# danini/progressive-x

Measured on AMD Instinct MI355X. Metric: residual_evals_per_sec, higher is better.
Workload: dtype f64; 1 GPU; C4 multi-6D-pose points (1e6 2D-3D correspondences, 16 objects, 20% outliers) x metric batch of 2048 pose hypotheses (16 GT + perturbed; weak mode: per GPU), PnP reprojection residual, MSAC + compound-model score, compound instance = 1 model; points=1000000, points_per_gpu=1000000, hypotheses_per_gpu=2048, hypotheses_total=2048, parallelism=1 GPU, exchange=none, device=AMD GPU, 256 CUs (gfx950:sramecc+:xnack-), cu_count=256

## Files before the change

### progressive-x_amd/csrc/score.hip

```cpp
#include <cmath>
#include <cstdlib>

#include "pgx_internal.h"
#include "score_filters.hip.h"
#include "score_runs.h"

namespace pgx {


template <int MT, bool MASK, int FILT>
__global__ __launch_bounds__(kScoreBlock) void score_kernel(
    const double* __restrict__ pts, int64_t n, const double* __restrict__ models, int M, int Mpad,
    double T2, const double* __restrict__ comp, int has_comp, int64_t chunk,
    const double* __restrict__ pmax, double guard, const float* __restrict__ pts32, double guard32,
    unsigned* __restrict__ pcnt, double* __restrict__ pval, double* __restrict__ psh,
    unsigned long long* __restrict__ masks, int64_t words, const int* __restrict__ perm, int chunks, int xcd_map,
    const float* __restrict__ gbounds)
{
    using R = Residual<MT>;
    int gx = (int)blockIdx.x, gy = (int)blockIdx.y;
    if (xcd_map) {
        const int groups = Mpad / kScoreBlock;
        const int slot = (int)(blockIdx.x >> 3);
        gx = slot % groups;
// ... 19 lines not shown
    const float Tup32 = f32_up(sqrt(T2) * (1.0 + 1.0 / 64.0));

    unsigned cnt = 0;
    double val = 0.0, sh = 0.0;
    unsigned long long word = 0;

    auto step = [&](int64_t i, const double (&pt)[R::D], double pm, const float* p32) {
        bool inl = false;
        bool rejected = false;
        if (FILT == 1 && F::enabled) rejected = F::reject(pt, mdl, flane, pm, T2d);
        if (FILT == 2 && F32::enabled) rejected = F32::reject(p32, flane32, T2d32);
        if (live && !rejected) {
            const double sq = R::squared(pt, mdl);
            inl = sq < T2;
            if (inl) {
                ++cnt;
                const double s = cv_max(0.0, 1.0 - sq / T2);
                val += s;
                if (has_comp) sh += cv_min(comp[i], s);
            }
        }
        if (MASK) {
            word |= (unsigned long long)(inl ? 1 : 0) << (i & 63);
            if ((i & 63) == 63 || i == i1 - 1) {
                if (live) masks[(int64_t)perm[m] * words + (i >> 6)] = word;
                word = 0;
            }
        }
    };
    constexpr int kUnroll = 4;
    int64_t i = i0;
    while (i < i1) {
        const int64_t gend = ((i | 63) + 1 < i1) ? (i | 63) + 1 : i1;
        if (FILT == 2 && F32::enabled && gbounds != nullptr) {
            const float* __restrict__ g = gbounds + (i >> 6) * kGroupRow;
            float gr[kGroupRow];
#pragma unroll
            for (int k = 0; k < 9; ++k) gr[k] = g[k];
            const bool keep = live && !F32::group_reject(gr, flane32, Tup32);
            if (__ballot(keep) == 0) {
                if (MASK && live) masks[(int64_t)perm[m] * words + (i >> 6)] = 0;
                i = gend;
                continue;
            }
        }
        for (; i + kUnroll <= gend; i += kUnroll) {
            const double* __restrict__ prow = pts + i * R::D;
            double pt[kUnroll][R::D];
            double pm[kUnroll];
            float p32[kUnroll][8];
#pragma unroll
            for (int u = 0; u < kUnroll; ++u) {
#pragma unroll
                for (int k = 0; k < R::D; ++k) pt[u][k] = prow[u * R::D + k];
                pm[u] = (FILT == 1 && F::enabled) ? pmax[i + u] : 1.0;
                if (FILT == 2 && F32::enabled) {
#pragma unroll
                    for (int k = 0; k < 8; ++k) p32[u][k] = pts32[(i + u) * 8 + k];
                }
            }
#pragma unroll
            for (int u = 0; u < kUnroll; ++u) step(i + u, pt[u], pm[u], p32[u]);
        }
        for (; i < gend; ++i) {
            const double* __restrict__ prow = pts + i * R::D;
            double pt[R::D];
            float p32[8];
#pragma unroll
            for (int k = 0; k < R::D; ++k) pt[k] = prow[k];
            if (FILT == 2 && F32::enabled) {
#pragma unroll
                for (int k = 0; k < 8; ++k) p32[k] = pts32[i * 8 + k];
            }
            step(i, pt, (FILT == 1 && F::enabled) ? pmax[i] : 1.0, p32);
        }
    }
    const int64_t o = (int64_t)gy * Mpad + m;
    pcnt[o] = cnt;
    pval[o] = val;
    psh[o] = sh;
}

#ifndef PGX_SCORE_TRIM
#define PGX_SCORE_TRIM 7
#endif
constexpr bool kTrimRows = (PGX_SCORE_TRIM & 1) != 0, kTrimDrain = (PGX_SCORE_TRIM & 2) != 0, kTrimDirect = (PGX_SCORE_TRIM & 4) != 0;

template <int MT> struct HypRow {
    using LaneT = typename Filter32<MT>::Lane;
    static_assert(sizeof(LaneT) % sizeof(float) == 0, "Filter32 lane constants are floats");
    static constexpr int kLaneVals = (int)(sizeof(LaneT) / sizeof(float));
    static constexpr int kVals = kTrimRows ? StagedVals<Filter32<MT>>::value : kLaneVals;
    static_assert(kVals <= kLaneVals, "the staged form is a prefix of the lane");
    static constexpr int kChunks = (kVals + 3) / 4;
    static constexpr int kStride = 4 * kChunks;

    static __device__ __forceinline__ void store(const LaneT& ln, float* __restrict__ row)
    {
        const float* src = reinterpret_cast<const float*>(&ln);
#pragma unroll
        for (int k = 0; k < kVals; ++k) row[k] = src[k];
    }
    static __device__ __forceinline__ LaneT load(const float* __restrict__ row)
    {
        LaneT ln;
        float* dst = reinterpret_cast<float*>(&ln);
#pragma unroll
        for (int k = 0; k < kVals; ++k) dst[k] = row[k];
        return ln;
    }
    static __device__ __forceinline__ void stage(const float* __restrict__ row0, float (*lds)[64][4], int lane)
    {
        const float* __restrict__ row = static_cast<const float*>(__builtin_assume_aligned(row0, 16));
#pragma unroll
        for (int c = 0; c < kChunks; ++c) {
            if (4 * c + 4 <= kVals) {
                *reinterpret_cast<float4*>(&lds[c][lane][0]) = *reinterpret_cast<const float4*>(row + 4 * c);
            } else {
#pragma unroll
                for (int k = 0; k < kVals - 4 * c; ++k) lds[c][lane][k] = row[4 * c + k];
            }
        }
    }
    static __device__ __forceinline__ LaneT staged(const float (*lds)[64][4], int h)
    {
        LaneT ln;
        float* dst = reinterpret_cast<float*>(&ln);
#pragma unroll
        for (int c = 0; c < kChunks; ++c) {
            if (4 * c + 4 <= kVals) {
                const float4 v = *reinterpret_cast<const float4*>(&lds[c][h][0]);
                dst[4 * c] = v.x; dst[4 * c + 1] = v.y; dst[4 * c + 2] = v.z; dst[4 * c + 3] = v.w;
            } else {
#pragma unroll
                for (int k = 0; k < kVals - 4 * c; ++k) dst[4 * c + k] = lds[c][h][k];
            }
        }
        return ln;
    }
};

constexpr int kCullWaves = 4;
constexpr int kCullTile = 64;

template <int MT>
__global__ __launch_bounds__(64 * kCullWaves) void score_cull_kernel(
    const double* __restrict__ models, int M, double T2, double guard32, const float* __restrict__ gbounds, int groups,
    int gps , int W, unsigned long long* __restrict__ keep, float* __restrict__ hyp32,
    double* __restrict__ models_t ,
    unsigned long long* __restrict__ zero , int64_t zero_words)
{
    using R = Residual<MT>;
    using F32 = Filter32<MT>;
    __shared__ __attribute__((aligned(16))) float s_gb[kCullTile + kCullTile / kSuper][kGroupRow];
    {
        const int64_t nthreads = (int64_t)gridDim.x * gridDim.y * (64 * kCullWaves);
        for (int64_t i = ((int64_t)blockIdx.y * gridDim.x + blockIdx.x) * (64 * kCullWaves) + threadIdx.x; i < zero_words; i += nthreads) zero[i] = 0ull;
    }
    const int lane = (int)(threadIdx.x & 63);
    const int w = (int)blockIdx.x * kCullWaves + (int)(threadIdx.x >> 6), seg = (int)blockIdx.y;
    const int m = w * 64 + lane;
    const bool live = w < W && m < M;
    double mdl[R::P];
#pragma unroll
    for (int k = 0; k < R::P; ++k) mdl[k] = live ? models[(int64_t)m * R::P + k] : __builtin_nan("");
    const typename F32::Lane flane32 = F32::prep(mdl, guard32, T2);
    if (seg == 0 && w < W) {
        HypRow<MT>::store(flane32, hyp32 + (int64_t)m * HypRow<MT>::kStride);
#pragma unroll
        for (int k = 0; k < R::P; ++k) models_t[(int64_t)k * W * 64 + m] = mdl[k];
    }
    const float Tup32 = f32_up(sqrt(T2) * (1.0 + 1.0 / 64.0));
    const int g0 = seg * gps, g1 = g0 + gps < groups ? g0 + gps : groups;
    for (int t0 = g0; t0 < g1; t0 += kCullTile) {
        const int cnt = g1 - t0 < kCullTile ? g1 - t0 : kCullTile;
        __syncthreads();
        const int scnt = (cnt + kSuper - 1) / kSuper;
        for (int e = (int)threadIdx.x; e < cnt * kGroupRow; e += 64 * kCullWaves)
            (&s_gb[0][0])[e] = gbounds[(int64_t)t0 * kGroupRow + e];
        for (int e = (int)threadIdx.x; e < scnt * kGroupRow; e += 64 * kCullWaves)
            (&s_gb[kCullTile][0])[e] = gbounds[((int64_t)groups + t0 / kSuper) * kGroupRow + e];
        __syncthreads();
        if (w >= W) continue;
        for (int sgi = 0; sgi < scnt; ++sgi) {
            const int i0 = sgi * kSuper, i1 = i0 + kSuper < cnt ? i0 + kSuper : cnt;
            float sr[kGroupRow];
#pragma unroll
            for (int k = 0; k < F32::kGroupVals; ++k) sr[k] = s_gb[kCullTile + sgi][k];
            if (__ballot(live && !F32::group_reject(sr, flane32, Tup32)) == 0) {
                if (lane < i1 - i0) keep[(int64_t)(t0 + i0 + lane) * W + w] = 0;
                continue;
            }
            for (int i = i0; i < i1; ++i) {
                float gr[kGroupRow];
#pragma unroll
                for (int k = 0; k < F32::kGroupVals; ++k) gr[k] = s_gb[i][k];
                const unsigned long long bm = __ballot(live && !F32::group_reject(gr, flane32, Tup32));
                if (lane == 0) keep[(int64_t)(t0 + i) * W + w] = bm;
            }
        }
    }
}

__device__ __forceinline__ long long to_fixed(double x)
{
    const double magic = 6755399441055744.0;
    return __double_as_longlong(x + magic) - __double_as_longlong(magic);
}

constexpr int kGroupWaves = 1;

template <int MT, bool MASK, bool STATS = false>
__global__ __launch_bounds__(64 * kGroupWaves) void score_group_kernel(
    const double* __restrict__ pts, const float* __restrict__ pts32, const double* __restrict__ comp, int64_t n, int groups,
    const double* __restrict__ models, int W, double T2, int has_comp, const unsigned long long* __restrict__ keep,
    const float* __restrict__ hyp32, double qscale, unsigned long long* __restrict__ acc ,
    int Mpad, unsigned long long* __restrict__ masks, int64_t words, const int* __restrict__ perm, int split, int xcd_local, const double* __restrict__ models_t,
    unsigned long long* __restrict__ stats ,
    const double* __restrict__ pts_g ,
    const float* __restrict__ p32_g , int nrep, int dense_min)
{
    using R = Residual<MT>;
    using F32 = Filter32<MT>;
    using LaneT = typename F32::Lane;
    using Row = HypRow<MT>;
    const int lane = (int)(threadIdx.x & 63);
    const int wv = 0;
    int g, part;
    if (xcd_local) {
        const int slot = (int)(blockIdx.x >> 3);
        g = (slot / split) * 8 + (int)(blockIdx.x & 7u);
        part = slot % split;
        if (g >= groups) return;
    } else {
        g = (int)blockIdx.x / split;
        part = (int)blockIdx.x % split;
    }
    g = __builtin_amdgcn_readfirstlane(g);
    part = __builtin_amdgcn_readfirstlane(part);
    {
        unsigned long long any = 0;
        for (int w = part; w < W; w += split) any |= keep[(int64_t)g * W + w];
        if (any == 0) return;
    }
    const int64_t j = (int64_t)g * 64 + lane;
    const bool valid = j < n;
    const int64_t jj = valid ? j : n - 1;
    double pt[R::D];
    float p32[8];
    if (pts_g != nullptr) {
#pragma unroll
        for (int q = 0; q < R::D; ++q) pt[q] = pts_g[((int64_t)g * R::D + q) * 64 + lane];
#pragma unroll
        for (int q = 0; q < 8; ++q) p32[q] = 0.0f;
        if constexpr (R::in1 >= R::in0) {
#pragma unroll
            for (int q = 0; q < R::D; ++q) p32[q] = (float)pt[q];
            double pm = 1.0;
#pragma unroll
            for (int q = R::in0; q <= R::in1; ++q) { const double a = fabs(pt[q]); if (!(a <= pm)) pm = a; }
            p32[5] = (float)(pm * 1.000001);
        } else {
#pragma unroll
            for (int q = 0; q < F32::kRowVals; ++q) p32[q] = p32_g[((int64_t)g * 8 + q) * 64 + lane];
        }
    } else {
#pragma unroll
        for (int q = 0; q < R::D; ++q) pt[q] = pts[jj * R::D + q];
#pragma unroll
        for (int q = 0; q < 8; ++q) p32[q] = pts32[jj * 8 + q];
    }
    const double cmp = has_comp ? comp[jj] : 0.0;
    acc += (size_t)(blockIdx.x % (unsigned)nrep) * 3 * (size_t)Mpad;
    const float T2d32 = f32_up(T2 * (1.0 + kFilter32Delta));
    __shared__ __attribute__((aligned(16))) float s_h32[kGroupWaves][Row::kChunks][64][4];
    __shared__ unsigned s_queue[kGroupWaves][128];
    int qn = 0;
    unsigned long long st_steps = 0, st_exact = 0, st_inl = 0;
    auto drain = [&](int c) __attribute__((always_inline)) {
        const bool act = lane < c;
        const unsigned e = act ? s_queue[wv][lane] : 0u;
        const int m = act ? (int)(e >> 6) : -1 - lane;
        const int src = act ? (int)(e & 63u) : lane;
        double q_pt[R::D];
#pragma unroll
        for (int k = 0; k < R::D; ++k) q_pt[k] = __shfl(pt[k], src, 64);
        const double q_cmp = has_comp ? __shfl(cmp, src, 64) : 0.0;
        long long cnt = 0, val = 0, shq = 0;
        if (act) {
            double mdl[R::P];
#pragma unroll
            for (int k = 0; k < R::P; ++k) mdl[k] = models_t[(int64_t)k * Mpad + m];
            const double sq = R::squared(q_pt, mdl);
            if (STATS) ++st_exact;
            if (sq < T2) {
                const double sc = cv_max(0.0, 1.0 - sq / T2);
                cnt = 1;
                if (STATS) ++st_inl;
                val = to_fixed(sc * qscale);
                if (has_comp) shq = to_fixed(cv_min(q_cmp, sc) * qscale);
            }
        }
        const int mp = __shfl_up(m, 1, 64);
        const bool head = lane == 0 || mp != m;
        if constexpr (kTrimDrain) {
            const int dist = run_dist(__ballot(head), lane);
            unsigned long long pv = run_pack((unsigned)cnt, (unsigned long long)val);
#pragma unroll 1
            for (int off = 1; off < 64; off <<= 1) {
                const bool same = off < dist;
                if (__ballot(same) == 0) break;
                const unsigned long long p2 = __shfl_down(pv, off, 64);
                if (same) pv += p2;
                if (has_comp) {
                    const long long s2 = __shfl_down(shq, off, 64);
                    if (same) shq += s2;
                }
            }
            cnt = (long long)run_count(pv);
            val = (long long)run_value(pv);
        } else {
            for (int off = 1; off < 64; off <<= 1) {
                const int mo = __shfl_down(m, off, 64);
                const bool same = lane + off < 64 && mo == m;
                if (__ballot(same) == 0) break;
                const long long c2 = __shfl_down(cnt, off, 64), v2 = __shfl_down(val, off, 64), s2 = __shfl_down(shq, off, 64);
                if (same) { cnt += c2; val += v2; shq += s2; }
            }
        }
        if (act && head && cnt > 0) {
            atomicAdd(&acc[m], (unsigned long long)cnt);
            atomicAdd(&acc[(int64_t)Mpad + m], (unsigned long long)val);
            if (has_comp) atomicAdd(&acc[2 * (int64_t)Mpad + m], (unsigned long long)shq);
        }
    };
    auto direct = [&](int m, bool cand) __attribute__((always_inline)) {
        double sc = 0.0, shv = 0.0;
        bool inl = false;
        if (cand) {
            double mdl[R::P];
#pragma unroll
            for (int k = 0; k < R::P; ++k) mdl[k] = models[(int64_t)m * R::P + k];
            const double sq = R::squared(pt, mdl);
            inl = sq < T2;
            if (STATS) { ++st_exact; if (inl) ++st_inl; }
            if (inl) {
                sc = cv_max(0.0, 1.0 - sq / T2);
                if (has_comp) shv = cv_min(cmp, sc);
            }
        }
        const unsigned long long bm = __ballot(inl);
        if (bm == 0) return;
        long long val = inl ? to_fixed(sc * qscale) : 0, shq = (inl && has_comp) ? to_fixed(shv * qscale) : 0;
        const bool shares = kTrimDirect ? (has_comp && __ballot(inl && shv != 0.0) != 0) : (has_comp != 0);
        if (shares) {
#pragma unroll
            for (int off = 32; off > 0; off >>= 1) {
                val += __shfl_down(val, off, 64);
                shq += __shfl_down(shq, off, 64);
            }
        } else {
#pragma unroll
            for (int off = 32; off > 0; off >>= 1) val += __shfl_down(val, off, 64);
        }
        if (lane == 0) {
            atomicAdd(&acc[m], (unsigned long long)__popcll(bm));
            atomicAdd(&acc[(int64_t)Mpad + m], (unsigned long long)val);
            if (shares) atomicAdd(&acc[2 * (int64_t)Mpad + m], (unsigned long long)shq);
            if (MASK) masks[(int64_t)perm[m] * words + g] = bm;
        }
    };
    for (int w = part; w < W; w += split) {
        unsigned long long todo = keep[(int64_t)g * W + w];
        if (todo == 0) continue;
        if (STATS) st_steps += (unsigned long long)__popcll(todo);
        __builtin_amdgcn_wave_barrier();
        if ((todo >> lane) & 1ull) {
            const int64_t ml = (int64_t)w * 64 + lane;
            Row::stage(hyp32 + ml * Row::kStride, s_h32[wv], lane);
        }
        __builtin_amdgcn_wave_barrier();
        while (todo != 0) {
            const int h = __builtin_ctzll(todo);
            todo &= todo - 1;
            const int m = w * 64 + h;
            const LaneT ln = Row::staged(s_h32[wv], h);
            const bool cand = valid && !F32::reject(p32, ln, T2d32);
            const unsigned long long cm = __ballot(cand);
            if (cm == 0) continue;
            if (!MASK && __popcll(cm) < dense_min) {
                if (cand) s_queue[wv][qn + __builtin_amdgcn_mbcnt_hi((unsigned)(cm >> 32), __builtin_amdgcn_mbcnt_lo((unsigned)cm, 0u))] =
                    ((unsigned)m << 6) | (unsigned)lane;
                qn += __popcll(cm);
                if (qn >= 64) {
                    __builtin_amdgcn_wave_barrier();
                    drain(64);
                    __builtin_amdgcn_wave_barrier();
                    const unsigned mv = s_queue[wv][64 + lane];
                    __builtin_amdgcn_wave_barrier();
                    s_queue[wv][lane] = mv;
                    qn -= 64;
                }
                continue;
            }
            direct(m, cand);
        }
    }
    if (!MASK && qn > 0) {
        __builtin_amdgcn_wave_barrier();
        drain(qn);
    }
    if (STATS) {
#pragma unroll
        for (int off = 32; off > 0; off >>= 1) {
            st_exact += __shfl_down(st_exact, off, 64);
            st_inl += __shfl_down(st_inl, off, 64);
        }
        if (lane == 0) {
            atomicAdd(&stats[0], st_steps);
            atomicAdd(&stats[1], st_exact);
            atomicAdd(&stats[2], st_inl);
        }
    }
}

template <int MT>
__global__ __launch_bounds__(64) void score_verify_kernel(const double* __restrict__ pts, const float* __restrict__ pts32, int64_t n,
                                                          const double* __restrict__ models, int M, int W, double T2,
                                                          const unsigned long long* __restrict__ keep, const float* __restrict__ hyp32,
                                                          unsigned long long* __restrict__ out)
{
    using R = Residual<MT>;
    using F32 = Filter32<MT>;
    using LaneT = typename F32::Lane;
    const int lane = (int)threadIdx.x, g = (int)blockIdx.x, w = (int)blockIdx.y;
    const int64_t j = (int64_t)g * 64 + lane;
    const bool valid = j < n;
    const int64_t jj = valid ? j : n - 1;
    double pt[R::D];
    float p32[8];
#pragma unroll
    for (int q = 0; q < R::D; ++q) pt[q] = pts[jj * R::D + q];
#pragma unroll
    for (int q = 0; q < 8; ++q) p32[q] = pts32[jj * 8 + q];
    const float T2d32 = f32_up(T2 * (1.0 + kFilter32Delta));
    const unsigned long long todo = keep[(int64_t)g * W + w];
    unsigned long long c_cull = 0, c_filt = 0, c_inl = 0;
    for (int h = 0; h < 64; ++h) {
        const int m = w * 64 + h;
        if (m >= M) break;
        double mdl[R::P];
#pragma unroll
        for (int k = 0; k < R::P; ++k) mdl[k] = models[(int64_t)m * R::P + k];
        const bool inl = valid && R::squared(pt, mdl) < T2;
        const bool kept = (todo >> h) & 1ull;
        const LaneT ln = HypRow<MT>::load(hyp32 + (int64_t)m * HypRow<MT>::kStride);
        const bool rej = F32::reject(p32, ln, T2d32);
        c_inl += inl;
        c_cull += inl && !kept;
        c_filt += inl && kept && rej;
    }
#pragma unroll
    for (int off = 32; off > 0; off >>= 1) {
        c_cull += __shfl_down(c_cull, off, 64);
        c_filt += __shfl_down(c_filt, off, 64);
        c_inl += __shfl_down(c_inl, off, 64);
    }
    if (lane == 0) {
        if (c_cull) atomicAdd(&out[0], c_cull);
        if (c_filt) atomicAdd(&out[1], c_filt);
        if (c_inl) atomicAdd(&out[2], c_inl);
    }
// ... 431 lines not shown
```

### progressive-x_amd/csrc/score_filters.hip.h

```cpp
#pragma once
#include <cmath>
#include <cstddef>
#include <type_traits>

#include "pgx_internal.h"

namespace pgx {

constexpr double kFilterDelta = 1.0 / 1048576.0;

template <int MT> struct Filter {
    static constexpr bool enabled = false;
    struct Lane {};
    template <class MD> static __device__ __forceinline__ Lane prep(const MD&, double) { return {}; }
    template <class PT, class MD>
    static __device__ __forceinline__ bool reject(const PT&, const MD&, const Lane&, double, double) { return false; }
};

template <> struct Filter<kPnP> {
    static constexpr bool enabled = true;
    struct Lane { double c; };
    template <class MD> static __device__ __forceinline__ Lane prep(const MD& m, double guard) {
        const double l0 = fabs(m[0]) + fabs(m[1]) + fabs(m[2]) + fabs(m[3]);
        const double l1 = fabs(m[4]) + fabs(m[5]) + fabs(m[6]) + fabs(m[7]);
        const double l2 = fabs(m[8]) + fabs(m[9]) + fabs(m[10]) + fabs(m[11]);
        const double l = fmax(l0, fmax(l1, l2));
        return {(l > 1e-100 && l < 1e100) ? guard * l : 1.0 / 0.0};
    }
    template <class PT, class MD>
    static __device__ __forceinline__ bool reject(const PT& p, const MD& m, const Lane& ln, double pmax, double T2d) {
        const double px = __builtin_fma(m[0], p[2], __builtin_fma(m[1], p[3], __builtin_fma(m[2], p[4], m[3])));
        const double py = __builtin_fma(m[4], p[2], __builtin_fma(m[5], p[3], __builtin_fma(m[6], p[4], m[7])));
        const double pz = __builtin_fma(m[8], p[2], __builtin_fma(m[9], p[3], __builtin_fma(m[10], p[4], m[11])));
        const double a = __builtin_fma(p[0], pz, -px);
        const double b = __builtin_fma(p[1], pz, -py);
        const double lhs = __builtin_fma(b, b, a * a);
        const double rhs = (pz * pz) * T2d;
        const bool trust = ln.c * pmax <= fabs(pz);
        return trust && (lhs > rhs);
    }
};

template <> struct Filter<kHomography> {
    static constexpr bool enabled = true;
    struct Lane { double c; };
    template <class MD> static __device__ __forceinline__ Lane prep(const MD& h, double guard) {
        const double l0 = fabs(h[0]) + fabs(h[1]) + fabs(h[2]);
        const double l1 = fabs(h[3]) + fabs(h[4]) + fabs(h[5]);
        const double l2 = fabs(h[6]) + fabs(h[7]) + fabs(h[8]);
        const double l = fmax(l0, fmax(l1, l2));
        return {(l > 1e-100 && l < 1e100) ? guard * l : 1.0 / 0.0};
    }
    template <class PT, class MD>
    static __device__ __forceinline__ bool reject(const PT& p, const MD& h, const Lane& ln, double pmax, double T2d) {
        const double t1 = __builtin_fma(h[0], p[0], __builtin_fma(h[1], p[1], h[2]));
        const double t2 = __builtin_fma(h[3], p[0], __builtin_fma(h[4], p[1], h[5]));
        const double t3 = __builtin_fma(h[6], p[0], __builtin_fma(h[7], p[1], h[8]));
        const double a = __builtin_fma(p[2], t3, -t1);
        const double b = __builtin_fma(p[3], t3, -t2);
        const double lhs = __builtin_fma(b, b, a * a);
        const double rhs = (t3 * t3) * T2d;
        const bool trust = ln.c * pmax <= fabs(t3);
        return trust && (lhs > rhs);
    }
};

template <> struct Filter<kHomographySym> : Filter<kHomography> {};

constexpr double kFilter32Delta = 1.0 / 128.0;
constexpr double kInflate = 1.000001;

__device__ __forceinline__ float f32_up(double x) { return (float)(x * kInflate); }

template <int P, class MD> __device__ __forceinline__ double pow2_normaliser(const MD& m, bool* off)
{
    double mx = 0.0;
#pragma unroll
    for (int k = 0; k < P; ++k) { const double a = fabs(m[k]); if (a > mx) mx = a; }
    *off = !(mx >= 1e-75) || !(mx <= 1e75);
    if (!(mx > 0.0) || !(mx < 1.7976931348623157e308)) return 1.0;
    int e;
    (void)frexp(mx, &e);
    return ldexp(1.0, -e);
}

template <int MT> struct Filter32 {
    static constexpr bool enabled = false;
    static constexpr int kRowVals = 6;
    static constexpr int kGroupVals = 9;
    struct Lane {};
    template <class MD> static __device__ __forceinline__ Lane prep(const MD&, double, double) { return {}; }
    static __device__ __forceinline__ bool reject(const float*, const Lane&, float) { return false; }
    static __device__ __forceinline__ bool group_reject(const float*, const Lane&, float) { return false; }
};

template <class F, class = void> struct StagedVals { static constexpr int value = (int)(sizeof(typename F::Lane) / sizeof(float)); };
template <class F> struct StagedVals<F, std::void_t<decltype(F::kStagedVals)>> { static constexpr int value = F::kStagedVals; };


template <> struct Filter32<kPnP> {
    static constexpr bool enabled = true;
    static constexpr int kRowVals = 6, kGroupVals = 9;
    struct Lane { float m[12]; float c1, c0; float n0, n1, n2; float nanh; };
    static constexpr int kStagedVals = 14;
    static_assert(offsetof(Lane, c0) == (kStagedVals - 1) * sizeof(float) && offsetof(Lane, n0) == kStagedVals * sizeof(float), "m, c1, c0 lead the lane");
    template <class MD> static __device__ __forceinline__ Lane prep(const MD& m0, double guard32, double) {
        Lane ln;
        bool nan = false;
        bool off;
        const double sc = pow2_normaliser<12>(m0, &off);
        double m[12];
#pragma unroll
        for (int k = 0; k < 12; ++k) { m[k] = m0[k] * sc; ln.m[k] = (float)m[k]; nan |= !(m0[k] == m0[k]); }
        ln.nanh = nan ? 1.0f : 0.0f;
        ln.n0 = (float)(sqrt(m[0] * m[0] + m[1] * m[1] + m[2] * m[2]) * kGroupInflate);
        ln.n1 = (float)(sqrt(m[4] * m[4] + m[5] * m[5] + m[6] * m[6]) * kGroupInflate);
        ln.n2 = (float)(sqrt(m[8] * m[8] + m[9] * m[9] + m[10] * m[10]) * kGroupInflate);
        const double l3 = fmax(fabs(m[0]) + fabs(m[1]) + fabs(m[2]),
                               fmax(fabs(m[4]) + fabs(m[5]) + fabs(m[6]), fabs(m[8]) + fabs(m[9]) + fabs(m[10])));
        const double t = fmax(fabs(m[3]), fmax(fabs(m[7]), fabs(m[11])));
        ln.c1 = f32_up(guard32 * l3);
        ln.c0 = off ? __builtin_inff() : fmaxf(f32_up(guard32 * t), 1e-30f);
        return ln;
    }
    static __device__ __forceinline__ bool reject(const float* p, const Lane& ln, float T2d) {
        const float* m = ln.m;
        const float px = __builtin_fmaf(m[0], p[2], __builtin_fmaf(m[1], p[3], __builtin_fmaf(m[2], p[4], m[3])));
        const float py = __builtin_fmaf(m[4], p[2], __builtin_fmaf(m[5], p[3], __builtin_fmaf(m[6], p[4], m[7])));
        const float pz = __builtin_fmaf(m[8], p[2], __builtin_fmaf(m[9], p[3], __builtin_fmaf(m[10], p[4], m[11])));
        const float a = __builtin_fmaf(p[0], pz, -px);
        const float b = __builtin_fmaf(p[1], pz, -py);
        const float lhs = __builtin_fmaf(b, b, a * a);
        const float rhs = (pz * pz) * T2d;
        const bool trust = __builtin_fmaf(ln.c1, p[5], ln.c0) <= fabsf(pz);
        return trust && (lhs > rhs);
    }
    static __device__ __forceinline__ bool group_reject(const float* g, const Lane& ln, float Tup) {
        const float* m = ln.m;
        const float cx = __builtin_fmaf(m[0], g[0], __builtin_fmaf(m[1], g[1], __builtin_fmaf(m[2], g[2], m[3])));
        const float cy = __builtin_fmaf(m[4], g[0], __builtin_fmaf(m[5], g[1], __builtin_fmaf(m[6], g[2], m[7])));
        const float cz = __builtin_fmaf(m[8], g[0], __builtin_fmaf(m[9], g[1], __builtin_fmaf(m[10], g[2], m[11])));
        if (ln.nanh != 0.0f) return true;
        const bool trust = __builtin_fmaf(ln.c1, g[8], ln.c0) <= fabsf(cz);
        const float dz = ln.n2 * g[3], dx = ln.n0 * g[3], dy = ln.n1 * g[3];
        const float zs = fabsf(cz) + dz;
        const float ex = fabsf(__builtin_fmaf(g[4], cz, -cx)), ey = fabsf(__builtin_fmaf(g[5], cz, -cy));
        const float mx = __builtin_fmaf(g[6], zs, __builtin_fmaf(fabsf(g[4]), dz, dx));
        const float my = __builtin_fmaf(g[7], zs, __builtin_fmaf(fabsf(g[5]), dz, dy));
        const float tol = Tup * zs;
        return trust && ((ex - mx > tol) || (ey - my > tol));
    }
};

template <> struct Filter32<kHomography> {
    static constexpr bool enabled = true;
    static constexpr int kRowVals = 6, kGroupVals = 9;
    struct Lane { float m[9]; float e1, e0; float n0, n1, n2; float nanh; };
    template <class MD> static __device__ __forceinline__ Lane prep(const MD& h0, double, double) {
        Lane ln;
        bool nan = false;
        bool off;
        const double sc = pow2_normaliser<9>(h0, &off);
        double h[9];
#pragma unroll
        for (int k = 0; k < 9; ++k) { h[k] = h0[k] * sc; ln.m[k] = (float)h[k]; nan |= !(h0[k] == h0[k]); }
        ln.nanh = nan ? 1.0f : 0.0f;
        ln.n0 = (float)(sqrt(h[0] * h[0] + h[1] * h[1]) * kGroupInflate);
        ln.n1 = (float)(sqrt(h[3] * h[3] + h[4] * h[4]) * kGroupInflate);
        ln.n2 = (float)(sqrt(h[6] * h[6] + h[7] * h[7]) * kGroupInflate);
        const double l2 = fmax(fabs(h[0]) + fabs(h[1]), fmax(fabs(h[3]) + fabs(h[4]), fabs(h[6]) + fabs(h[7])));
        const double t = fmax(fabs(h[2]), fmax(fabs(h[5]), fabs(h[8])));
        const double u = 5.9604644775390625e-8, eta = 1.1754943508222875e-38;
        ln.e1 = f32_up(5.5 * u * l2 + 4.0 * eta);
        ln.e0 = off ? __builtin_inff() : f32_up(5.5 * u * t + eta);
        return ln;
    }
    static __device__ __forceinline__ bool reject(const float* p, const Lane& ln, float T2d) {
        const float* h = ln.m;
        const float t1 = __builtin_fmaf(h[0], p[0], __builtin_fmaf(h[1], p[1], h[2]));
        const float t2 = __builtin_fmaf(h[3], p[0], __builtin_fmaf(h[4], p[1], h[5]));
        const float t3 = __builtin_fmaf(h[6], p[0], __builtin_fmaf(h[7], p[1], h[8]));
        const float a = fabsf(__builtin_fmaf(p[2], t3, -t1));
        const float b = fabsf(__builtin_fmaf(p[3], t3, -t2));
        const float Et = __builtin_fmaf(ln.e1, p[5], ln.e0);
        const float at3 = fabsf(t3);
        const float base = __builtin_fmaf(6.0202e-8f  * p[5], at3, __builtin_fmaf(Et, p[5], Et));
        const float ma = fmaxf(a - __builtin_fmaf(6.0202e-8f, a, base), 0.0f);
        const float mb = fmaxf(b - __builtin_fmaf(6.0202e-8f, b, base), 0.0f);
        const float den = at3 + Et;
        return __builtin_fmaf(mb, mb, ma * ma) > (den * den) * T2d && (base == base);
    }
    static __device__ __forceinline__ bool group_reject(const float* g, const Lane& ln, float Tup) {
        const float* h = ln.m;
        const float cx = __builtin_fmaf(h[0], g[0], __builtin_fmaf(h[1], g[1], h[2]));
        const float cy = __builtin_fmaf(h[3], g[0], __builtin_fmaf(h[4], g[1], h[5]));
        const float cz = __builtin_fmaf(h[6], g[0], __builtin_fmaf(h[7], g[1], h[8]));
        if (ln.nanh != 0.0f) return true;
        const float Et = __builtin_fmaf(ln.e1, g[8], ln.e0);
        const float dz = ln.n2 * g[3], dx = ln.n0 * g[3], dy = ln.n1 * g[3];
        const float acz = fabsf(cz);
        const float zs = acz + dz + Et;
        const float ex = fabsf(__builtin_fmaf(g[4], cz, -cx)), ey = fabsf(__builtin_fmaf(g[5], cz, -cy));
        const float aub = fabsf(g[4]), avb = fabsf(g[5]);
        const float Egx = __builtin_fmaf(Et, aub, Et) + 6.0202e-8f * __builtin_fmaf(aub, acz, ex);
        const float Egy = __builtin_fmaf(Et, avb, Et) + 6.0202e-8f * __builtin_fmaf(avb, acz, ey);
        const float mx = __builtin_fmaf(g[6], zs, __builtin_fmaf(aub, dz, dx)) + Egx;
        const float my = __builtin_fmaf(g[7], zs, __builtin_fmaf(avb, dz, dy)) + Egy;
        const float tol = Tup * zs;
        return (ex - mx * 1.0001f > tol) || (ey - my * 1.0001f > tol);
    }
};

template <> struct Filter32<kVanishingPoint> {
    static constexpr bool enabled = true;
    static constexpr int kRowVals = 7, kGroupVals = 12;
    struct Lane { float v[3]; float e2, e1, e0, e50, t2pp, invT, nanh; };
    template <class MD> static __device__ __forceinline__ Lane prep(const MD& v0, double, double T2) {
        Lane ln;
        bool off;
        const double sc = pow2_normaliser<3>(v0, &off);
        const double v[3] = {v0[0] * sc, v0[1] * sc, v0[2] * sc};
        ln.v[0] = (float)v[0]; ln.v[1] = (float)v[1]; ln.v[2] = (float)v[2];
        ln.nanh = (v0[0] == v0[0] && v0[1] == v0[1] && v0[2] == v0[2]) ? 0.0f : 1.0f;
        const double V1 = fabs(v[0]) + fabs(v[1]), V2 = fabs(v[2]), T = sqrt(T2);
        const double k38 = 3.637978807091713e-12 , k11 = 4.8828125e-4 ;
        ln.e2 = f32_up(k38 * V2 / T * 1.001);
        ln.e1 = f32_up((k11 * V2 + k38 * V1 / T) * 1.001);
        ln.e0 = off ? __builtin_inff() : fmaxf(f32_up(k11 * V1 * 1.001), 1e-37f);
        ln.e50 = f32_up(8.881784197001252e-16  * V2 * 1.001);
        ln.t2pp = f32_up(T2 * (1.0 + 1.0 / 64.0));
        ln.invT = (float)(1.0 / (T * (1.0 + 1.0 / 64.0)) * 0.99999);
        return ln;
    }
    static __device__ __forceinline__ bool reject(const float* p, const Lane& ln, float) {
        const float* v = ln.v;
        const float N = __builtin_fmaf(v[0], p[0], __builtin_fmaf(v[1], p[1], v[2] * p[2]));
        const float S = __builtin_fmaf(fabsf(v[0]), fabsf(p[0]), __builtin_fmaf(fabsf(v[1]), fabsf(p[1]), fabsf(v[2]) * fabsf(p[2])));
        const float lx = __builtin_fmaf(p[4], v[2], -v[1]);
        const float ly = __builtin_fmaf(-p[3], v[2], v[0]);
        const float D2 = __builtin_fmaf(lx, lx, ly * ly);
        const float tt = __builtin_fmaf(ln.e2, p[6], __builtin_fmaf(ln.e1, p[5], ln.e0));
        const float m = fabsf(N) - __builtin_fmaf(4.76837158203125e-7f , S, ln.e50 * p[6]);
        return (D2 >= tt * tt) && (m > 0.0f) && (m * m > ln.t2pp * D2);
    }
    static __device__ __forceinline__ bool group_reject(const float* g, const Lane& ln, float) {
        const float* v = ln.v;
        if (ln.nanh != 0.0f) return true;
        const float N = __builtin_fmaf(v[0], g[0], __builtin_fmaf(v[1], g[1], v[2] * g[2]));
        const float S = __builtin_fmaf(fabsf(v[0]), fabsf(g[0]), __builtin_fmaf(fabsf(v[1]), fabsf(g[1]), fabsf(v[2]) * fabsf(g[2])));
        const float RN = __builtin_fmaf(fabsf(v[0]), g[5], __builtin_fmaf(fabsf(v[1]), g[6], fabsf(v[2]) * g[7]));
        const float lx = __builtin_fmaf(g[4], v[2], -v[1]);
        const float ly = __builtin_fmaf(-g[3], v[2], v[0]);
        const float D2 = __builtin_fmaf(lx, lx, ly * ly);
        const float RD = fabsf(v[2]) * g[8] * 1.001f;
        const float tt0 = __builtin_fmaf(ln.e2, g[11], __builtin_fmaf(ln.e1, g[10], ln.e0));
        const float tt = tt0 + RD;
        const float L = fabsf(N) - RN * 1.001f - 1.9073486328125e-6f  * S;
        const float G = L * g[9] * ln.invT - RD;
        const bool trust = (D2 >= tt * tt * 1.001f) || (L >= tt0 * 1.01f);
        return trust && (G > 0.0f) && (G * G > D2 * 1.004f);
    }
};

template <> struct Filter32<kFundamental> {
    static constexpr bool enabled = true;
    static constexpr int kRowVals = 7, kGroupVals = 9;
    struct Lane { float f[9]; float e1, e0, n2, n1, n0, t2pp, nA, nanh; };
    template <class MD> static __device__ __forceinline__ Lane prep(const MD& f0, double pscale2 , double T2) {
        Lane ln;
        bool nan = false, big = false;
        bool off;
        const double sc = pow2_normaliser<9>(f0, &off);
        big = off;
        double f[9];
#pragma unroll
        for (int k = 0; k < 9; ++k) { f[k] = f0[k] * sc; ln.f[k] = (float)f[k]; nan |= !(f0[k] == f0[k]); big |= !(fabs(f[k]) * pscale2 <= 1e36); }
        ln.nanh = nan ? 1.0f : 0.0f;
        const double A4 = fabs(f[0]) + fabs(f[1]) + fabs(f[3]) + fabs(f[4]), B4 = fabs(f[2]) + fabs(f[5]) + fabs(f[6]) + fabs(f[7]);
        const double u = 5.9604644775390625e-8, eta = 1.1754943508222875e-38, itau = 1024.0;
        ln.e1 = f32_up((4.1 * u * 2.0 * A4 + 8.0 * eta) * itau);
        ln.e0 = big ? __builtin_inff() : fmaxf(f32_up(4.1 * u * B4 * itau), 1e-12f);
        ln.n2 = f32_up(8.5 * u * A4 + 16.0 * eta);
        ln.n1 = f32_up(8.5 * u * B4);
        ln.n0 = f32_up(8.5 * u * fabs(f[8]));
        ln.t2pp = f32_up(T2 * (1.0 + 1.0 / 64.0));
        ln.nA = f32_up(sqrt(f[0] * f[0] + f[1] * f[1] + f[3] * f[3] + f[4] * f[4]) * 1.001);
        return ln;
    }
    static __device__ __forceinline__ bool reject(const float* p, const Lane& ln, float) {
        const float* f = ln.f;
        const float rxc = __builtin_fmaf(f[0], p[2], __builtin_fmaf(f[3], p[3], f[6]));
        const float ryc = __builtin_fmaf(f[1], p[2], __builtin_fmaf(f[4], p[3], f[7]));
        const float rwc = __builtin_fmaf(f[2], p[2], __builtin_fmaf(f[5], p[3], f[8]));
        const float n = __builtin_fmaf(p[0], rxc, __builtin_fmaf(p[1], ryc, rwc));
        const float rx = __builtin_fmaf(f[0], p[0], __builtin_fmaf(f[1], p[1], f[2]));
        const float ry = __builtin_fmaf(f[3], p[0], __builtin_fmaf(f[4], p[1], f[5]));
        const float D2 = __builtin_fmaf(rxc, rxc, __builtin_fmaf(ryc, ryc, __builtin_fmaf(rx, rx, ry * ry)));
        const float tt = __builtin_fmaf(ln.e1, p[5], ln.e0);
        const float m = fabsf(n) - __builtin_fmaf(ln.n2, p[6], __builtin_fmaf(ln.n1, p[5], ln.n0));
        return (D2 >= tt * tt) && (m > 0.0f) && (m * m > ln.t2pp * D2);
    }
    static __device__ __forceinline__ bool group_reject(const float* g, const Lane& ln, float Tup) {
        const float* f = ln.f;
        if (ln.nanh != 0.0f) return true;
        const float rxc = __builtin_fmaf(f[0], g[2], __builtin_fmaf(f[3], g[3], f[6]));
        const float ryc = __builtin_fmaf(f[1], g[2], __builtin_fmaf(f[4], g[3], f[7]));
        const float rwc = __builtin_fmaf(f[2], g[2], __builtin_fmaf(f[5], g[3], f[8]));
        const float n = __builtin_fmaf(g[0], rxc, __builtin_fmaf(g[1], ryc, rwc));
        const float rx = __builtin_fmaf(f[0], g[0], __builtin_fmaf(f[1], g[1], f[2]));
        const float ry = __builtin_fmaf(f[3], g[0], __builtin_fmaf(f[4], g[1], f[5]));
        const float D2 = __builtin_fmaf(rxc, rxc, __builtin_fmaf(ryc, ryc, __builtin_fmaf(rx, rx, ry * ry)));
        const float ED = __builtin_fmaf(ln.e1, g[7], ln.e0) * 9.765625e-4f ;
        const float G = __builtin_sqrtf(D2) * 1.001f + ED;
        const float En = __builtin_fmaf(ln.n2, g[8], __builtin_fmaf(ln.n1, g[7], ln.n0));
        const float L = fabsf(n) - En - (G * g[6] + ln.nA * g[4] * g[5]) * 1.001f;
        const float U = __builtin_fmaf(ln.nA, g[6], G) * 1.001f;
        return L > Tup * U;
    }
};

template <> struct Filter32<kHomographySym> : Filter32<kHomography> {
    template <class MD> static __device__ __forceinline__ Lane prep(const MD& h, double guard32, double T2) {
        Lane ln = Filter32<kHomography>::prep(h, guard32, T2);
        bool nan = false;
#pragma unroll
        for (int k = 0; k < 18; ++k) nan |= !(h[k] == h[k]);
        ln.nanh = nan ? 1.0f : 0.0f;
        return ln;
    }
};

template <> struct Filter32<kLine2D> {
    static constexpr bool enabled = true;
    static constexpr int kRowVals = 6, kGroupVals = 4;
    struct Lane { float a, b, c, e1, e0, nrm, tpp, nanh; };
    template <class MD> static __device__ __forceinline__ Lane prep(const MD& m0, double pscale , double T2) {
        Lane ln;
        bool off;
        const double sc = pow2_normaliser<3>(m0, &off);
        const double m[3] = {m0[0] * sc, m0[1] * sc, m0[2] * sc};
        ln.a = (float)m[0]; ln.b = (float)m[1]; ln.c = (float)m[2];
        ln.nanh = (m0[0] == m0[0] && m0[1] == m0[1] && m0[2] == m0[2]) ? 0.0f : 1.0f;
        const double Ts = sqrt(T2) * sc;
        const bool big = !(fabs(m[0]) * pscale <= 1e36) || !(fabs(m[1]) * pscale <= 1e36) || !(fabs(m[2]) <= 1e36) || !(Ts > 1e-30) || !(Ts < 1e30) || off;
        const double u = 5.9604644775390625e-8, eta = 1.1754943508222875e-38;
        ln.e1 = f32_up(4.1 * u * (fabs(m[0]) + fabs(m[1])) + 4.0 * eta);
        ln.e0 = big ? __builtin_inff() : f32_up(4.1 * u * fabs(m[2]) + eta);
        ln.nrm = f32_up(sqrt(m[0] * m[0] + m[1] * m[1]) * 1.001);
        ln.tpp = f32_up(Ts * (1.0 + 1.0 / 64.0));
        return ln;
    }
    static __device__ __forceinline__ bool reject(const float* p, const Lane& ln, float) {
        const float n = __builtin_fmaf(ln.a, p[0], __builtin_fmaf(ln.b, p[1], ln.c));
        const float m = fabsf(n) - __builtin_fmaf(ln.e1, p[5], ln.e0);
        return m > ln.tpp;
    }
    static __device__ __forceinline__ bool group_reject(const float* g, const Lane& ln, float) {
        if (ln.nanh != 0.0f) return true;
        const float n = __builtin_fmaf(ln.a, g[0], __builtin_fmaf(ln.b, g[1], ln.c));
        const float m = fabsf(n) - __builtin_fmaf(ln.e1, g[3], ln.e0) - ln.nrm * g[2] * 1.001f;
        return m > ln.tpp * 1.001f;
    }
};

template <> struct Filter32<kPlane3D> {
    static constexpr bool enabled = true;
    static constexpr int kRowVals = 6, kGroupVals = 5;
    struct Lane { float a, b, c, d, e1, e0, nrm, tpp, nanh; };
    template <class MD> static __device__ __forceinline__ Lane prep(const MD& m0, double pscale , double T2) {
        Lane ln;
        bool off;
        const double sc = pow2_normaliser<4>(m0, &off);
        const double m[4] = {m0[0] * sc, m0[1] * sc, m0[2] * sc, m0[3] * sc};
        ln.a = (float)m[0]; ln.b = (float)m[1]; ln.c = (float)m[2]; ln.d = (float)m[3];
        ln.nanh = (m0[0] == m0[0] && m0[1] == m0[1] && m0[2] == m0[2] && m0[3] == m0[3]) ? 0.0f : 1.0f;
        const double Ts = sqrt(T2) * sc;
        const bool big = !(fabs(m[0]) * pscale <= 1e36) || !(fabs(m[1]) * pscale <= 1e36) || !(fabs(m[2]) * pscale <= 1e36) ||
                         !(fabs(m[3]) <= 1e36) || !(Ts > 1e-30) || !(Ts < 1e30) || off;
        const double u = 5.9604644775390625e-8, eta = 1.1754943508222875e-38;
        ln.e1 = f32_up(5.1 * u * (fabs(m[0]) + fabs(m[1]) + fabs(m[2])) + 6.0 * eta);
        ln.e0 = big ? __builtin_inff() : f32_up(5.1 * u * fabs(m[3]) + 4.0 * eta);
        ln.nrm = f32_up(sqrt(m[0] * m[0] + m[1] * m[1] + m[2] * m[2]) * 1.001);
        ln.tpp = f32_up(Ts * (1.0 + 1.0 / 64.0));
        return ln;
    }
    static __device__ __forceinline__ bool reject(const float* p, const Lane& ln, float) {
        const float n = __builtin_fmaf(ln.a, p[0], __builtin_fmaf(ln.b, p[1], __builtin_fmaf(ln.c, p[2], ln.d)));
        const float m = fabsf(n) - __builtin_fmaf(ln.e1, p[5], ln.e0);
        return m > ln.tpp;
    }
    static __device__ __forceinline__ bool group_reject(const float* g, const Lane& ln, float) {
        if (ln.nanh != 0.0f) return true;
        const float n = __builtin_fmaf(ln.a, g[0], __builtin_fmaf(ln.b, g[1], __builtin_fmaf(ln.c, g[2], ln.d)));
        const float m = fabsf(n) - __builtin_fmaf(ln.e1, g[4], ln.e0) - ln.nrm * g[3] * 1.001f;
        return m > ln.tpp * 1.001f;
    }
};

template <> struct Filter32<kSphere3D> {
    static constexpr bool enabled = true;
    static constexpr int kRowVals = 6, kGroupVals = 5;
    struct Lane { float cx, cy, cz, r, e1, e0, e2, tpp, nanh; };
    template <class MD> static __device__ __forceinline__ Lane prep(const MD& m, double pscale , double T2) {
        Lane ln;
        ln.cx = (float)m[0]; ln.cy = (float)m[1]; ln.cz = (float)m[2]; ln.r = (float)m[3];
        ln.nanh = (m[0] == m[0] && m[1] == m[1] && m[2] == m[2] && m[3] == m[3]) ? 0.0f : 1.0f;
        const double Ts = sqrt(T2);
        const double cn = sqrt((m[0] * m[0] + m[1] * m[1]) + m[2] * m[2]) * 1.001;
        const bool big = !(pscale <= 1e17) || !(cn <= 1e17) || !(fabs(m[3]) <= 1e17) || !(Ts > 1e-30) || !(Ts < 1e30);
        const double u = 5.9604644775390625e-8;
        ln.e1 = f32_up(2.0 * u);
        ln.e0 = big ? __builtin_inff() : f32_up(2.0 * u * (cn + fabs(m[3])) + 1e-18);
        ln.e2 = f32_up(8.0 * u);
        ln.tpp = f32_up(Ts * (1.0 + 1.0 / 64.0));
        return ln;
    }
    static __device__ __forceinline__ float dist(const float* p, const Lane& ln) {
        const float dx = p[0] - ln.cx, dy = p[1] - ln.cy, dz = p[2] - ln.cz;
        return sqrtf(__builtin_fmaf(dx, dx, __builtin_fmaf(dy, dy, dz * dz)));
    }
    static __device__ __forceinline__ bool reject(const float* p, const Lane& ln, float) {
        const float s = dist(p, ln);
        const float m = fabsf(s - ln.r) - (__builtin_fmaf(ln.e1, p[5], ln.e0) + ln.e2 * s);
        return m > ln.tpp;
    }
    static __device__ __forceinline__ bool group_reject(const float* g, const Lane& ln, float) {
        if (ln.nanh != 0.0f) return true;
        const float s = dist(g, ln);
        const float m = fabsf(s - ln.r) - (__builtin_fmaf(ln.e1, g[4], ln.e0) + ln.e2 * (s + g[3])) - g[3] * 1.001f;
        return m > ln.tpp * 1.001f;
    }
};

template <> struct Filter32<kCircle2D> {
    static constexpr bool enabled = true;
    static constexpr int kRowVals = 6, kGroupVals = 4;
    struct Lane { float cx, cy, r, e1, e0, e2, tpp, nanh; };
    template <class MD> static __device__ __forceinline__ Lane prep(const MD& m, double pscale , double T2) {
        Lane ln;
        ln.cx = (float)m[0]; ln.cy = (float)m[1]; ln.r = (float)m[2];
        ln.nanh = (m[0] == m[0] && m[1] == m[1] && m[2] == m[2]) ? 0.0f : 1.0f;
        const double Ts = sqrt(T2);
        const double cn = sqrt(m[0] * m[0] + m[1] * m[1]) * 1.001;
        const bool big = !(pscale <= 1e17) || !(cn <= 1e17) || !(fabs(m[2]) <= 1e17) || !(Ts > 1e-30) || !(Ts < 1e30);
        const double u = 5.9604644775390625e-8;
        ln.e1 = f32_up(2.0 * u);
        ln.e0 = big ? __builtin_inff() : f32_up(2.0 * u * (cn + fabs(m[2])) + 1e-18);
        ln.e2 = f32_up(8.0 * u);
        ln.tpp = f32_up(Ts * (1.0 + 1.0 / 64.0));
        return ln;
    }
    static __device__ __forceinline__ float dist(const float* p, const Lane& ln) {
        const float dx = p[0] - ln.cx, dy = p[1] - ln.cy;
        return sqrtf(__builtin_fmaf(dx, dx, dy * dy));
    }
    static __device__ __forceinline__ bool reject(const float* p, const Lane& ln, float) {
        const float s = dist(p, ln);
        const float m = fabsf(s - ln.r) - (__builtin_fmaf(ln.e1, p[5], ln.e0) + ln.e2 * s);
        return m > ln.tpp;
    }
    static __device__ __forceinline__ bool group_reject(const float* g, const Lane& ln, float) {
        if (ln.nanh != 0.0f) return true;
        const float s = dist(g, ln);
        const float m = fabsf(s - ln.r) - (__builtin_fmaf(ln.e1, g[3], ln.e0) + ln.e2 * (s + g[2])) - g[2] * 1.001f;
        return m > ln.tpp * 1.001f;
    }
};

}
```

Baseline: 11210 billion residual-evals/s.

## Reload drained points from memory, use scalar-base gathers and wave-mask filter rejects

Three trim flags are added and turned on by default. In the drain path, each queued lane now reloads its point and compound value from global memory through a wave-uniform scalar base and a 32-bit offset, instead of shuffling R::D doubles across lanes. Model parameters are gathered the same way. The per-hypothesis filter test now builds the candidate mask directly from per-condition ballots, so the wave gets the mask without a per-lane bool followed by a ballot. This is meant to cut cross-lane shuffle traffic and 64-bit address arithmetic, at the cost of extra global or cache loads in the drain.

Measured after the change: 11070 billion residual-evals/s. 0.988x the previous value.

```diff
diff --git a/progressive-x_amd/csrc/score.hip b/progressive-x_amd/csrc/score.hip
--- a/progressive-x_amd/csrc/score.hip
+++ b/progressive-x_amd/csrc/score.hip
@@ -125,9 +125,10 @@
 }
 
 #ifndef PGX_SCORE_TRIM
-#define PGX_SCORE_TRIM 7
+#define PGX_SCORE_TRIM 63
 #endif
 constexpr bool kTrimRows = (PGX_SCORE_TRIM & 1) != 0, kTrimDrain = (PGX_SCORE_TRIM & 2) != 0, kTrimDirect = (PGX_SCORE_TRIM & 4) != 0;
+constexpr bool kTrimPoint = (PGX_SCORE_TRIM & 8) != 0, kTrimGather = (PGX_SCORE_TRIM & 16) != 0, kTrimMask = (PGX_SCORE_TRIM & 32) != 0;
 
 template <int MT> struct HypRow {
     using LaneT = typename Filter32<MT>::Lane;
@@ -251,6 +252,25 @@
     return __double_as_longlong(x + magic) - __double_as_longlong(magic);
 }
 
+using GlobalBytes = const __attribute__((address_space(1))) char*;
+template <class T>
+__device__ __forceinline__ GlobalBytes uniform_base(const T* p)
+{
+    const unsigned long long a = reinterpret_cast<unsigned long long>(p);
+    const unsigned lo = __builtin_amdgcn_readfirstlane((unsigned)a), hi = __builtin_amdgcn_readfirstlane((unsigned)(a >> 32));
+    return reinterpret_cast<GlobalBytes>(((unsigned long long)hi << 32) | lo);
+}
+__device__ __forceinline__ double load_f64(GlobalBytes base, unsigned byte_offset)
+{
+    return *reinterpret_cast<const __attribute__((address_space(1))) double*>(base + byte_offset);
+}
+
+__device__ __forceinline__ unsigned long long wave_ballot(bool p)
+{
+    if constexpr (kTrimMask) return __builtin_amdgcn_ballot_w64(p);
+    else return __ballot(p);
+}
+
 constexpr int kGroupWaves = 1;
 
 template <int MT, bool MASK, bool STATS = false>
@@ -289,6 +309,8 @@
     const int64_t j = (int64_t)g * 64 + lane;
     const bool valid = j < n;
     const int64_t jj = valid ? j : n - 1;
+    const int64_t nvalid = n - (int64_t)g * 64;
+    const unsigned long long valid_mask = nvalid >= 64 ? ~0ull : nvalid > 0 ? (1ull << nvalid) - 1ull : 0ull;
     double pt[R::D];
     float p32[8];
     if (pts_g != nullptr) {
@@ -326,14 +348,38 @@
         const int m = act ? (int)(e >> 6) : -1 - lane;
         const int src = act ? (int)(e & 63u) : lane;
         double q_pt[R::D];
-#pragma unroll
-        for (int k = 0; k < R::D; ++k) q_pt[k] = __shfl(pt[k], src, 64);
-        const double q_cmp = has_comp ? __shfl(cmp, src, 64) : 0.0;
+        double q_cmp = 0.0;
+        if constexpr (!kTrimPoint) {
+#pragma unroll
+            for (int k = 0; k < R::D; ++k) q_pt[k] = __shfl(pt[k], src, 64);
+            if (has_comp) q_cmp = __shfl(cmp, src, 64);
+        }
         long long cnt = 0, val = 0, shq = 0;
         if (act) {
+            if constexpr (kTrimPoint) {
+                const unsigned so = (unsigned)src * 8u;
+                if (pts_g != nullptr) {
+                    const GlobalBytes pb = uniform_base(pts_g + (int64_t)g * R::D * 64);
+#pragma unroll
+                    for (int k = 0; k < R::D; ++k) q_pt[k] = load_f64(pb, so + (unsigned)k * 512u);
+                } else {
+                    const double* __restrict__ pr = pts + ((int64_t)g * 64 + src) * R::D;
+#pragma unroll
+                    for (int k = 0; k < R::D; ++k) q_pt[k] = pr[k];
+                    __builtin_amdgcn_wave_barrier();
+                }
+                if (has_comp) q_cmp = load_f64(uniform_base(comp + (int64_t)g * 64), so);
+            }
             double mdl[R::P];
-#pragma unroll
-            for (int k = 0; k < R::P; ++k) mdl[k] = models_t[(int64_t)k * Mpad + m];
+            if constexpr (kTrimGather) {
+                const unsigned mo = (unsigned)m * 8u;
+#pragma unroll
+                for (int k = 0; k < R::P; ++k)
+                    mdl[k] = load_f64(uniform_base(models_t + (int64_t)k * Mpad), mo);
+            } else {
+#pragma unroll
+                for (int k = 0; k < R::P; ++k) mdl[k] = models_t[(int64_t)k * Mpad + m];
+            }
             const double sq = R::squared(q_pt, mdl);
             if (STATS) ++st_exact;
             if (sq < T2) {
@@ -347,12 +393,12 @@
         const int mp = __shfl_up(m, 1, 64);
         const bool head = lane == 0 || mp != m;
         if constexpr (kTrimDrain) {
-            const int dist = run_dist(__ballot(head), lane);
+            const int dist = run_dist(wave_ballot(head), lane);
             unsigned long long pv = run_pack((unsigned)cnt, (unsigned long long)val);
 #pragma unroll 1
             for (int off = 1; off < 64; off <<= 1) {
                 const bool same = off < dist;
-                if (__ballot(same) == 0) break;
+                if (wave_ballot(same) == 0) break;
                 const unsigned long long p2 = __shfl_down(pv, off, 64);
                 if (same) pv += p2;
                 if (has_comp) {
@@ -392,10 +438,10 @@
                 if (has_comp) shv = cv_min(cmp, sc);
             }
         }
-        const unsigned long long bm = __ballot(inl);
+        const unsigned long long bm = wave_ballot(inl);
         if (bm == 0) return;
         long long val = inl ? to_fixed(sc * qscale) : 0, shq = (inl && has_comp) ? to_fixed(shv * qscale) : 0;
-        const bool shares = kTrimDirect ? (has_comp && __ballot(inl && shv != 0.0) != 0) : (has_comp != 0);
+        const bool shares = kTrimDirect ? (has_comp && wave_ballot(inl && shv != 0.0) != 0) : (has_comp != 0);
         if (shares) {
 #pragma unroll
             for (int off = 32; off > 0; off >>= 1) {
@@ -428,9 +474,17 @@
             todo &= todo - 1;
             const int m = w * 64 + h;
             const LaneT ln = Row::staged(s_h32[wv], h);
-            const bool cand = valid && !F32::reject(p32, ln, T2d32);
-            const unsigned long long cm = __ballot(cand);
-            if (cm == 0) continue;
+            bool cand;
+            unsigned long long cm;
+            if constexpr (kTrimMask) {
+                cm = ~F32::template reject_as<WaveAll>(p32, ln, T2d32) & valid_mask;
+                if (cm == 0) continue;
+                cand = ((cm >> lane) & 1ull) != 0;
+            } else {
+                cand = valid && !F32::reject(p32, ln, T2d32);
+                cm = __ballot(cand);
+                if (cm == 0) continue;
+            }
             if (!MASK && __popcll(cm) < dense_min) {
                 if (cand) s_queue[wv][qn + __builtin_amdgcn_mbcnt_hi((unsigned)(cm >> 32), __builtin_amdgcn_mbcnt_lo((unsigned)cm, 0u))] =
                     ((unsigned)m << 6) | (unsigned)lane;
diff --git a/progressive-x_amd/csrc/score_filters.hip.h b/progressive-x_amd/csrc/score_filters.hip.h
--- a/progressive-x_amd/csrc/score_filters.hip.h
+++ b/progressive-x_amd/csrc/score_filters.hip.h
@@ -84,12 +84,20 @@
     return ldexp(1.0, -e);
 }
 
+struct LaneAll {
+    template <class... B> static __device__ __forceinline__ bool all(B... b) { return (b && ...); }
+};
+struct WaveAll {
+    template <class... B> static __device__ __forceinline__ unsigned long long all(B... b) { return (__builtin_amdgcn_ballot_w64(b) & ...); }
+};
+
 template <int MT> struct Filter32 {
     static constexpr bool enabled = false;
     static constexpr int kRowVals = 6;
     static constexpr int kGroupVals = 9;
     struct Lane {};
     template <class MD> static __device__ __forceinline__ Lane prep(const MD&, double, double) { return {}; }
+    template <class C> static __device__ __forceinline__ auto reject_as(const float*, const Lane&, float) { return C::all(false); }
     static __device__ __forceinline__ bool reject(const float*, const Lane&, float) { return false; }
     static __device__ __forceinline__ bool group_reject(const float*, const Lane&, float) { return false; }
 };
@@ -123,7 +131,7 @@
         ln.c0 = off ? __builtin_inff() : fmaxf(f32_up(guard32 * t), 1e-30f);
         return ln;
     }
-    static __device__ __forceinline__ bool reject(const float* p, const Lane& ln, float T2d) {
+    template <class C> static __device__ __forceinline__ auto reject_as(const float* p, const Lane& ln, float T2d) {
         const float* m = ln.m;
         const float px = __builtin_fmaf(m[0], p[2], __builtin_fmaf(m[1], p[3], __builtin_fmaf(m[2], p[4], m[3])));
         const float py = __builtin_fmaf(m[4], p[2], __builtin_fmaf(m[5], p[3], __builtin_fmaf(m[6], p[4], m[7])));
@@ -133,8 +141,9 @@
         const float lhs = __builtin_fmaf(b, b, a * a);
         const float rhs = (pz * pz) * T2d;
         const bool trust = __builtin_fmaf(ln.c1, p[5], ln.c0) <= fabsf(pz);
-        return trust && (lhs > rhs);
-    }
+        return C::all(trust, lhs > rhs);
+    }
+    static __device__ __forceinline__ bool reject(const float* p, const Lane& ln, float T2d) { return reject_as<LaneAll>(p, ln, T2d); }
     static __device__ __forceinline__ bool group_reject(const float* g, const Lane& ln, float Tup) {
         const float* m = ln.m;
         const float cx = __builtin_fmaf(m[0], g[0], __builtin_fmaf(m[1], g[1], __builtin_fmaf(m[2], g[2], m[3])));
@@ -175,7 +184,7 @@
         ln.e0 = off ? __builtin_inff() : f32_up(5.5 * u * t + eta);
         return ln;
     }
-    static __device__ __forceinline__ bool reject(const float* p, const Lane& ln, float T2d) {
+    template <class C> static __device__ __forceinline__ auto reject_as(const float* p, const Lane& ln, float T2d) {
         const float* h = ln.m;
         const float t1 = __builtin_fmaf(h[0], p[0], __builtin_fmaf(h[1], p[1], h[2]));
         const float t2 = __builtin_fmaf(h[3], p[0], __builtin_fmaf(h[4], p[1], h[5]));
@@ -188,8 +197,9 @@
         const float ma = fmaxf(a - __builtin_fmaf(6.0202e-8f, a, base), 0.0f);
         const float mb = fmaxf(b - __builtin_fmaf(6.0202e-8f, b, base), 0.0f);
         const float den = at3 + Et;
-        return __builtin_fmaf(mb, mb, ma * ma) > (den * den) * T2d && (base == base);
-    }
+        return C::all(__builtin_fmaf(mb, mb, ma * ma) > (den * den) * T2d, base == base);
+    }
+    static __device__ __forceinline__ bool reject(const float* p, const Lane& ln, float T2d) { return reject_as<LaneAll>(p, ln, T2d); }
     static __device__ __forceinline__ bool group_reject(const float* g, const Lane& ln, float Tup) {
         const float* h = ln.m;
         const float cx = __builtin_fmaf(h[0], g[0], __builtin_fmaf(h[1], g[1], h[2]));
@@ -232,7 +242,7 @@
         ln.invT = (float)(1.0 / (T * (1.0 + 1.0 / 64.0)) * 0.99999);
         return ln;
     }
-    static __device__ __forceinline__ bool reject(const float* p, const Lane& ln, float) {
+    template <class C> static __device__ __forceinline__ auto reject_as(const float* p, const Lane& ln, float) {
         const float* v = ln.v;
         const float N = __builtin_fmaf(v[0], p[0], __builtin_fmaf(v[1], p[1], v[2] * p[2]));
         const float S = __builtin_fmaf(fabsf(v[0]), fabsf(p[0]), __builtin_fmaf(fabsf(v[1]), fabsf(p[1]), fabsf(v[2]) * fabsf(p[2])));
@@ -241,8 +251,9 @@
         const float D2 = __builtin_fmaf(lx, lx, ly * ly);
         const float tt = __builtin_fmaf(ln.e2, p[6], __builtin_fmaf(ln.e1, p[5], ln.e0));
         const float m = fabsf(N) - __builtin_fmaf(4.76837158203125e-7f , S, ln.e50 * p[6]);
-        return (D2 >= tt * tt) && (m > 0.0f) && (m * m > ln.t2pp * D2);
-    }
+        return C::all(D2 >= tt * tt, m > 0.0f, m * m > ln.t2pp * D2);
+    }
+    static __device__ __forceinline__ bool reject(const float* p, const Lane& ln, float T2d) { return reject_as<LaneAll>(p, ln, T2d); }
     static __device__ __forceinline__ bool group_reject(const float* g, const Lane& ln, float) {
         const float* v = ln.v;
         if (ln.nanh != 0.0f) return true;
@@ -287,7 +298,7 @@
         ln.nA = f32_up(sqrt(f[0] * f[0] + f[1] * f[1] + f[3] * f[3] + f[4] * f[4]) * 1.001);
         return ln;
     }
-    static __device__ __forceinline__ bool reject(const float* p, const Lane& ln, float) {
+    template <class C> static __device__ __forceinline__ auto reject_as(const float* p, const Lane& ln, float) {
         const float* f = ln.f;
         const float rxc = __builtin_fmaf(f[0], p[2], __builtin_fmaf(f[3], p[3], f[6]));
         const float ryc = __builtin_fmaf(f[1], p[2], __builtin_fmaf(f[4], p[3], f[7]));
@@ -298,8 +309,9 @@
         const float D2 = __builtin_fmaf(rxc, rxc, __builtin_fmaf(ryc, ryc, __builtin_fmaf(rx, rx, ry * ry)));
         const float tt = __builtin_fmaf(ln.e1, p[5], ln.e0);
         const float m = fabsf(n) - __builtin_fmaf(ln.n2, p[6], __builtin_fmaf(ln.n1, p[5], ln.n0));
-        return (D2 >= tt * tt) && (m > 0.0f) && (m * m > ln.t2pp * D2);
-    }
+        return C::all(D2 >= tt * tt, m > 0.0f, m * m > ln.t2pp * D2);
+    }
+    static __device__ __forceinline__ bool reject(const float* p, const Lane& ln, float T2d) { return reject_as<LaneAll>(p, ln, T2d); }
     static __device__ __forceinline__ bool group_reject(const float* g, const Lane& ln, float Tup) {
         const float* f = ln.f;
         if (ln.nanh != 0.0f) return true;
@@ -350,11 +362,12 @@
         ln.tpp = f32_up(Ts * (1.0 + 1.0 / 64.0));
         return ln;
     }
-    static __device__ __forceinline__ bool reject(const float* p, const Lane& ln, float) {
+    template <class C> static __device__ __forceinline__ auto reject_as(const float* p, const Lane& ln, float) {
         const float n = __builtin_fmaf(ln.a, p[0], __builtin_fmaf(ln.b, p[1], ln.c));
         const float m = fabsf(n) - __builtin_fmaf(ln.e1, p[5], ln.e0);
-        return m > ln.tpp;
-    }
+        return C::all(m > ln.tpp);
+    }
+    static __device__ __forceinline__ bool reject(const float* p, const Lane& ln, float T2d) { return reject_as<LaneAll>(p, ln, T2d); }
     static __device__ __forceinline__ bool group_reject(const float* g, const Lane& ln, float) {
         if (ln.nanh != 0.0f) return true;
         const float n = __builtin_fmaf(ln.a, g[0], __builtin_fmaf(ln.b, g[1], ln.c));
@@ -384,11 +397,12 @@
         ln.tpp = f32_up(Ts * (1.0 + 1.0 / 64.0));
         return ln;
     }
-    static __device__ __forceinline__ bool reject(const float* p, const Lane& ln, float) {
+    template <class C> static __device__ __forceinline__ auto reject_as(const float* p, const Lane& ln, float) {
         const float n = __builtin_fmaf(ln.a, p[0], __builtin_fmaf(ln.b, p[1], __builtin_fmaf(ln.c, p[2], ln.d)));
         const float m = fabsf(n) - __builtin_fmaf(ln.e1, p[5], ln.e0);
-        return m > ln.tpp;
-    }
+        return C::all(m > ln.tpp);
+    }
+    static __device__ __forceinline__ bool reject(const float* p, const Lane& ln, float T2d) { return reject_as<LaneAll>(p, ln, T2d); }
     static __device__ __forceinline__ bool group_reject(const float* g, const Lane& ln, float) {
         if (ln.nanh != 0.0f) return true;
         const float n = __builtin_fmaf(ln.a, g[0], __builtin_fmaf(ln.b, g[1], __builtin_fmaf(ln.c, g[2], ln.d)));
@@ -419,11 +433,12 @@
         const float dx = p[0] - ln.cx, dy = p[1] - ln.cy, dz = p[2] - ln.cz;
         return sqrtf(__builtin_fmaf(dx, dx, __builtin_fmaf(dy, dy, dz * dz)));
     }
-    static __device__ __forceinline__ bool reject(const float* p, const Lane& ln, float) {
+    template <class C> static __device__ __forceinline__ auto reject_as(const float* p, const Lane& ln, float) {
         const float s = dist(p, ln);
         const float m = fabsf(s - ln.r) - (__builtin_fmaf(ln.e1, p[5], ln.e0) + ln.e2 * s);
-        return m > ln.tpp;
-    }
+        return C::all(m > ln.tpp);
+    }
+    static __device__ __forceinline__ bool reject(const float* p, const Lane& ln, float T2d) { return reject_as<LaneAll>(p, ln, T2d); }
     static __device__ __forceinline__ bool group_reject(const float* g, const Lane& ln, float) {
         if (ln.nanh != 0.0f) return true;
         const float s = dist(g, ln);
@@ -454,11 +469,12 @@
         const float dx = p[0] - ln.cx, dy = p[1] - ln.cy;
         return sqrtf(__builtin_fmaf(dx, dx, dy * dy));
     }
-    static __device__ __forceinline__ bool reject(const float* p, const Lane& ln, float) {
+    template <class C> static __device__ __forceinline__ auto reject_as(const float* p, const Lane& ln, float) {
         const float s = dist(p, ln);
         const float m = fabsf(s - ln.r) - (__builtin_fmaf(ln.e1, p[5], ln.e0) + ln.e2 * s);
-        return m > ln.tpp;
-    }
+        return C::all(m > ln.tpp);
+    }
+    static __device__ __forceinline__ bool reject(const float* p, const Lane& ln, float T2d) { return reject_as<LaneAll>(p, ln, T2d); }
     static __device__ __forceinline__ bool group_reject(const float* g, const Lane& ln, float) {
         if (ln.nanh != 0.0f) return true;
         const float s = dist(g, ln);
```
